# Saguaro-Biosciences/image-processing-suite

Measured on AMD Instinct MI355X. Metric: fields-of-view/sec, 2080x2080x5ch illum+seg+feat pipe, higher is better.
Workload: dtype fp32 planes / fp64 QC+features / fp32 CPnet (split-fp16 MFMA, f16x3); 1 GPU; configs[1]: 384-well plate, 1 FOV/well, 2080x2080x5ch, illum->seg->feat; batch_per_gpu=48, H=2080, W=2080, C=5, cellpose_model=nuclei, cpnet_weights=cpnet_nuclei_synth.pt, tiles_per_fov=9, parallelism=fov-sharded x1, scheduler=static per-rank steps, steps_this_rank=30, batches_in_flight_per_gpu=2

## Files before the change

### image-processing-suite_amd/csrc/cpx_internal.h

```cpp
#pragma once
#include <hip/hip_runtime.h>
#include <stdint.h>
#include <stddef.h>
#include <string>
#include <algorithm>
#include "../../include/cpx.h"

constexpr int kWsSlots = 16;

struct cpx_fov_state;

struct cpx_ctx {
  int device = 0;
  hipStream_t own_stream = nullptr;
  hipStream_t stream = nullptr;
  void* ws[kWsSlots] = {nullptr};
  size_t ws_bytes[kWsSlots] = {0};
  unsigned int ws_gen[kWsSlots] = {0};
  int n_cu = 256;
  int qc_H = 0, qc_W = 0;
  unsigned int qc_gen = 0;
  int seg_key[6] = {0, 0, 0, 0, 0, 0};
  unsigned int seg_gen = 0;
  cpx_fov_state* fov = nullptr;
// ... 64 lines not shown
template <typename T>
__device__ __forceinline__ T wave_sum(T v) {
#pragma unroll
  for (int off = 32; off > 0; off >>= 1) v += __shfl_xor(v, off, 64);
  return v;
}
template <typename T>
__device__ __forceinline__ T wave_min(T v) {
#pragma unroll
  for (int off = 32; off > 0; off >>= 1) {
    T o = __shfl_xor(v, off, 64);
    v = o < v ? o : v;
  }
  return v;
}
template <typename T>
__device__ __forceinline__ T wave_max(T v) {
#pragma unroll
  for (int off = 32; off > 0; off >>= 1) {
    T o = __shfl_xor(v, off, 64);
    v = o > v ? o : v;
  }
  return v;
}

constexpr int kClaimBroken = 1 << 30;

constexpr int kFeRegMaxLong = 128, kFeRegMaxShort = 120;
constexpr int kFeRegRows = 40;
constexpr int kFeReg1Rows = 80;
constexpr int kFeKS = 12;
constexpr int kFeU = 1;
constexpr int kFeLargeThreads = 1024, kFeLargeCells = 20224;
__host__ __device__ constexpr int fe_stride(int bw) { return (bw + 3) & ~1; }
__host__ __device__ constexpr bool fe_fits(int bh, int bw, int threads, int units, int cells) {
  const int nsr = (bh + kFeKS - 1) / kFeKS;
  return (long long)(bh + 2) * fe_stride(bw) <= cells &&
         (long long)((bw + 1) / 2) * nsr <= (long long)threads * units;
}
__host__ __device__ constexpr int fe_reg_class(int bh, int bw, bool& tr) {
  const int mn = bh < bw ? bh : bw, mx = bh < bw ? bw : bh;
  if (mn < 1) return 0;
  if (mx <= 64) { tr = bh > bw; return 1; }
  if (mn <= 64 && mx <= kFeReg1Rows) { tr = bw > bh; return 1; }
  if (mx <= 128 && mn <= 2 * kFeRegRows) { tr = bh > bw; return 2; }
  if (mx <= 128 && mn <= 3 * kFeRegRows) { tr = bh > bw; return 3; }
  return 0;
}
enum { kFeListReg1 = 0, kFeListReg2, kFeListReg3, kFeListLds, kFeListOver, kFeListUnd, kFeListFallback, kFeLists };
struct cpx_fe_lists {
  int* count;
  int2* items;
  long long cap;
  __device__ __forceinline__ int n(int l) const { return count[l]; }
  __device__ __forceinline__ int2 at(int l, int i) const { return items[l * cap + i]; }
  __device__ __forceinline__ void push(int l, int fov, int kobj) const {
    items[l * cap + atomicAdd(&count[l], 1)] = make_int2(fov, kobj);
  }
};
__host__ __device__ constexpr int fe_class(int bh, int bw) {
  bool tr = false;
  const int c = fe_reg_class(bh, bw, tr);
  if (c) return kFeListReg1 + c - 1;
  return fe_fits(bh, bw, kFeLargeThreads / 2, 2 * kFeU, kFeLargeCells) ? kFeListLds : kFeListOver;
}
static_assert(fe_class(kFeRegMaxLong, kFeRegMaxShort) == kFeListReg3 &&
                  fe_fits(kFeRegMaxLong, kFeRegMaxShort, kFeLargeThreads / 2, 2 * kFeU, kFeLargeCells) &&
                  fe_fits(kFeRegMaxShort, kFeRegMaxLong, kFeLargeThreads / 2, 2 * kFeU, kFeLargeCells),
              "register-class masks must fit the LDS screening class");

constexpr int kFastShapeWords = 4096;
__host__ __device__ inline bool cpx_shape_fits(int bh, int bw) {
  return (bh + 4) * ((bw + 4 + 31) >> 5) <= kFastShapeWords;
}
struct cpx_fallback_lists {
  int* shape;
  int* tex;
  int* n_shape;
  int* n_tex;
};
typedef int (*cpx_fallback_fn)(cpx_ctx* ctx, hipStream_t stream, const cpx_fallback_lists& fb,
                               void* arg);
int cpx_flow_error_reg_launch(int n_cu, hipStream_t stream, const int* m0, const float2* dpf, int Dy, int Dx,
                              int ML, const cpx_object* obj, cpx_fe_lists lists, int* ctr, double thr,
                              unsigned char* bad);
int cpx_features_fast(cpx_ctx* ctx, const int32_t* labels_dev, const float* corr_dev, int B, int C,
                      int H, int W, int max_label, int F, const cpx_object* objects_dev,
                      const cpx_fov_objects* hdr_dev, double* feats_dev, cpx_fallback_lists* fb,
                      cpx_fallback_fn fallback, void* fallback_arg);
int cpx_features_pair_fast(cpx_ctx* ctx, const int32_t* labels_dev, const int32_t* tlabels_dev,
                           const float* corr_dev, int B, int C, int H, int W, int max_label, int F,
                           const cpx_object* objects_dev, const cpx_fov_objects* hdr_dev, double* feats_dev,
                           const cpx_object* tobjects_dev, const cpx_fov_objects* thdr_dev, double* tfeats_dev,
                           cpx_fallback_lists* fb, cpx_fallback_lists* tfb);
```

### image-processing-suite_amd/csrc/k_flowerr_reg.hip

```cpp
#include "cpx_internal.h"
#include <math.h>
#include <stdlib.h>


#pragma clang fp contract(off)

namespace {

__device__ __forceinline__ float dpp_from_left(float v) {
  return __int_as_float(__builtin_amdgcn_mov_dpp(__float_as_int(v), 0x138, 0xf, 0xf, true));
}
__device__ __forceinline__ float dpp_from_right(float v) {
  return __int_as_float(__builtin_amdgcn_mov_dpp(__float_as_int(v), 0x130, 0xf, 0xf, true));
}

__device__ __forceinline__ int fe_hist_rank(const int* h, int len, long long k) {
  const int lane = threadIdx.x & 63;
  int e[3], s = 0;
#pragma unroll
  for (int u = 0; u < 3; ++u) {
    e[u] = 3 * lane + u < len ? h[3 * lane + u] : 0;
    s += e[u];
  }
#pragma unroll
  for (int d = 1; d < 64; d <<= 1) {
    const int y = __shfl_up(s, d, 64);
    if (lane >= d) s += y;
  }
  const unsigned long long bb = __ballot((long long)s > k);
  const int lb = bb ? __ffsll((long long)bb) - 1 : 63;
  const long long c0 = (long long)__shfl(s - e[1] - e[2], lb, 64);
  const long long c1 = c0 + __shfl(e[1], lb, 64);
  return c0 > k ? 3 * lb : c1 > k ? 3 * lb + 1 : 3 * lb + 2;
}

static_assert(3 * kFeRegRows == kFeRegMaxShort && 2 * 64 == kFeRegMaxLong, "cpx_internal.h class bounds");
typedef float fe_v2 __attribute__((ext_vector_type(2)));

template <int OP, int RW, int LO = 0, typename V>
__device__ __forceinline__ void fe_row_op(V* T, int jc, V& v) {
  if constexpr (RW - LO == 1) {
    if (jc == LO) {
      if constexpr (OP == 0) T[LO] += v;
      if constexpr (OP == 1) T[LO] = v;
      if constexpr (OP == 2) v = T[LO];
      asm volatile("; fe_row_op %0 %1" ::"n"(OP), "n"(LO));
    }
  } else {
    constexpr int MID = LO + (RW - LO) / 2;
    if (jc < MID) fe_row_op<OP, MID, LO, V>(T, jc, v);
    else fe_row_op<OP, RW, MID, V>(T, jc, v);
  }
}

constexpr int kFeReg3Rows = 32;
static_assert(4 * kFeReg3Rows >= kFeRegMaxShort, "class 3 rows fit four waves");

template <int RW, int NW, int CLS>
__global__ __launch_bounds__(64 * NW, 2) void k_flow_error_reg(
    const int* __restrict__ m0, const float2* __restrict__ dpf, int Dy, int Dx, int max_label,
    const cpx_object* __restrict__ objects, cpx_fe_lists lists, int* __restrict__ ctr, double thr,
    unsigned char* __restrict__ bad) {
  static_assert(RW % 8 == 0, "rows in groups of 8");
  constexpr int NT = 64 * NW;
  __shared__ fe_v2 xr[2][NW][2][64];
  __shared__ int hrow[RW * NW], hcol[128];
  __shared__ double sred[NW][3];
  __shared__ unsigned long long sbest[NW];
  __shared__ int sitem, smed2[2];
  const int tid = threadIdx.x, lane = tid & 63, wv = tid >> 6;
  const long long n = (long long)Dy * Dx;
  constexpr int kList = kFeListReg1 + CLS - 1;
  const int total = lists.n(kList);
  for (int claims = 0;; ++claims) {
    if (claims > total) {
      if (tid == 0) atomicOr(ctr, kClaimBroken);
      break;
    }
    if (tid == 0) sitem = atomicAdd(ctr, 1);
    __syncthreads();
    const int item = __builtin_amdgcn_readfirstlane(sitem);
    __syncthreads();
    if (item >= total) break;
    const int2 code = lists.at(kList, item);
    const int fov = code.x, kobj = code.y;
    const cpx_object o = objects[(long long)fov * max_label + kobj];
    const int L = o.label;
    const int r0 = o.bbox[0], c0 = o.bbox[1];
    const int bh = o.bbox[2] - r0, bw = o.bbox[3] - c0;
    bool tr = false;
    fe_reg_class(bh, bw, tr);
    const int SR = tr ? bw : bh, SC = tr ? bh : bw;
    const int RS = (SR + NW - 1) / NW;
    const int nrow = __builtin_amdgcn_readfirstlane(max(0, min(RS, SR - wv * RS)));
    const int* lab = m0 + (long long)fov * n + (long long)r0 * Dx + c0;
    for (int i = tid; i < RW * NW; i += NT) hrow[i] = 0;
    for (int i = tid; i < 128; i += NT) hcol[i] = 0;
    __syncthreads();
    fe_v2 T[RW], Wt[RW];
    const int gca = 2 * lane + 1, gcb = 2 * lane + 2;
    const bool ca_in = gca <= SC, cb_in = gcb <= SC;
    const int offa = tr ? (gca - 1) * Dx : gca - 1, offb = tr ? (gcb - 1) * Dx : gcb - 1;
    const int rstep = tr ? 1 : Dx;
// ... 317 lines not shown
      }
#pragma unroll
      for (int k = 0; k + 8 < RW; ++k) {
        T[k] = T[k + 8];
        Wt[k] = Wt[k + 8];
      }
#pragma unroll
      for (int k = RW - 8; k < RW; ++k) {
        T[k] = 0.f;
        Wt[k] = 0.f;
      }
    }
    e0 = wave_sum(e0);
    e1 = wave_sum(e1);
    eb = wave_sum(eb);
    if (lane == 0) {
      const double err = 0.0 + e0 / (double)o.area + e1 / (double)o.area;
      const double bnd = eb / (double)o.area + 1e-9 * (1.0 + err);
      const unsigned char v = err - thr > bnd ? 1 : thr - err > bnd ? 2 : 3;
      if (v == 3) lists.push(kFeListUnd, fov, kobj);
      bad[(long long)fov * (max_label + 1) + L] = v;
    }
  }
}


}

int cpx_flow_error_reg_launch(int n_cu, hipStream_t stream, const int* m0, const float2* dpf, int Dy, int Dx,
                              int ML, const cpx_object* obj, cpx_fe_lists lists, int* ctr, double thr,
                              unsigned char* bad) {
  hipLaunchKernelGGL((k_flow_error_reg1<kFeReg1Rows>), dim3(8 * n_cu), dim3(64), 0, stream, m0, dpf, Dy, Dx,
                     ML, obj, lists, ctr, thr, bad);
  hipLaunchKernelGGL((k_flow_error_reg<kFeRegRows, 2, 2>), dim3(4 * n_cu), dim3(128), 0, stream, m0, dpf, Dy, Dx,
                     ML, obj, lists, ctr + 1, thr, bad);
  hipLaunchKernelGGL((k_flow_error_reg<kFeReg3Rows, 4, 3>), dim3(2 * n_cu), dim3(256), 0, stream, m0, dpf, Dy, Dx,
                     ML, obj, lists, ctr + 2, thr, bad);
  CPX_CHECK_LAUNCH("k_flow_error_reg");
  return CPX_OK;
}
```

### image-processing-suite_amd/csrc/k_seg.hip

```cpp
#include "cpx_internal.h"
#include <stdlib.h>
#include <limits.h>
#include <math.h>
#include <stdio.h>
#include <type_traits>
#include <vector>

#pragma clang fp contract(off)

namespace {

constexpr int kT = 256;
constexpr int kRpad = 20;

__device__ __forceinline__ unsigned int f2key(float f) {
  unsigned int u = __float_as_uint(f);
  return (u & 0x80000000u) ? ~u : (u | 0x80000000u);
}
__device__ __forceinline__ float key2f(unsigned int k) {
  unsigned int u = (k & 0x80000000u) ? (k & 0x7fffffffu) : ~k;
  return __uint_as_float(u);
}
__device__ __forceinline__ unsigned short f2bf16(float f) {
  unsigned int u = __float_as_uint(f);
  if ((u & 0x7fffffffu) > 0x7f800000u) return 0x7fc0;
  u += 0x7fffu + ((u >> 16) & 1u);
  return (unsigned short)(u >> 16);
}
__device__ __forceinline__ float bf162f(unsigned short h) {
  return __uint_as_float(((unsigned int)h) << 16);
}

struct PctState {
// ... 823 lines not shown
  for (int j = blockIdx.x * kT + threadIdx.x; j < n_masks; j += gridDim.x * kT) {
    const int pix = d.marklist[(long long)fov * d.ms + j];
    d.mark[(long long)fov * n + pix] = 0;
    d.newlab[(long long)fov * (d.ms + 1) + d.m0[(long long)fov * n + pix]] = j + 1;
  }
  if (blockIdx.x == 0 && threadIdx.x == 0) d.st[fov].n_masks = n_masks;
}

__global__ __launch_bounds__(kT) void k_apply_newlab(int Dy, int Dx, DynBufs d) {
  const int fov = blockIdx.y;
  const long long n = (long long)Dy * Dx;
  const long long q0 = ((long long)blockIdx.x * kT + threadIdx.x) * kPx4;
  if (q0 >= n) return;
  int* m = d.m0 + (long long)fov * n;
  const int* nl = d.newlab + (long long)fov * (d.ms + 1);
  if ((n & 3) == 0 && (((uintptr_t)d.m0) & 15u) == 0) {
    const int4 t = *reinterpret_cast<const int4*>(m + q0);
    int4 o;
    o.x = t.x ? nl[t.x] : 0;
    o.y = t.y ? nl[t.y] : 0;
    o.z = t.z ? nl[t.z] : 0;
    o.w = t.w ? nl[t.w] : 0;
    *reinterpret_cast<int4*>(m + q0) = o;
  } else {
#pragma unroll
    for (int u = 0; u < kPx4; ++u)
      if (q0 + u < n) {
        const int l = m[q0 + u];
        m[q0 + u] = l ? nl[l] : 0;
      }
  }
}

template <typename E, typename E2>
__device__ __forceinline__ void fe_pair(const E2& ua, const E2& ub, const E2& ca, const E2& cb, const E2& da,
                                        const E2& db, E& n0, E& n1) {
  E s0 = ca.y + ua.y, s1 = cb.x + ub.x;
  s0 = s0 + da.y;
  s1 = s1 + db.x;
  s0 = s0 + ca.x;
  s1 = s1 + ca.y;
  s0 = s0 + cb.x;
  s1 = s1 + cb.y;
  s0 = s0 + ua.x;
  s1 = s1 + ua.y;
  s0 = s0 + ub.x;
  s1 = s1 + ub.y;
  s0 = s0 + da.x;
  s1 = s1 + da.y;
  s0 = s0 + db.x;
  s1 = s1 + db.y;
  n0 = (E)(1 / 9.) * s0;
  n1 = (E)(1 / 9.) * s1;
}

static_assert(kFeKS <= 32, "unit mask bits");

__global__ __launch_bounds__(256) void k_fe_classify(int max_label, const cpx_object* __restrict__ objects,
                                                     const cpx_fov_objects* __restrict__ hdr,
                                                     cpx_fe_lists lists) {
  const int fov = blockIdx.y, k = blockIdx.x * 256 + threadIdx.x, lane = threadIdx.x & 63;
  int cls = -1;
  if (k < min(hdr[fov].n_objects, max_label)) {
    const cpx_object& o = objects[(long long)fov * max_label + k];
    cls = fe_class(o.bbox[2] - o.bbox[0], o.bbox[3] - o.bbox[1]);
  }
  for (int c = kFeListReg1; c <= kFeListOver; ++c) {
    const unsigned long long b = __ballot(cls == c);
    if (!b) continue;
    const int lead = __ffsll((long long)b) - 1;
    int base = 0;
    if (lane == lead) base = atomicAdd(&lists.count[c], __popcll(b));
    base = __shfl(base, lead, 64);
    if (cls == c) lists.items[c * lists.cap + base + __popcll(b & ((1ull << lane) - 1ull))] = make_int2(fov, k);
  }
}

template <int THREADS>
struct FeShared {
  double sred[THREADS / 64][3];
  unsigned long long sbest[THREADS / 64];
  double smed[2];
  int sitem, stot;
};

template <int THREADS, int U, typename E>
__device__ __forceinline__ void fe_lds_mask(E* T, FeShared<THREADS>& sh, const int* __restrict__ m0,
                                            const float2* __restrict__ dpf, int Dy, int Dx, int max_label,
                                            const cpx_object* __restrict__ objects, const cpx_fe_lists& lists,
                                            int fov, int kobj, double thr, unsigned char* __restrict__ bad) {
  constexpr bool kScreen = std::is_same<E, float>::value;
  typedef typename std::conditional<kScreen, float2, double2>::type E2;
  auto& sred = sh.sred;
  auto& sbest = sh.sbest;
  auto& smed = sh.smed;
  const long long n = (long long)Dy * Dx;
  const int tid = threadIdx.x, lane = tid & 63, wid = tid >> 6;
  {
    const cpx_object o = objects[(long long)fov * max_label + kobj];
    const int L = o.label;
    const int r0 = o.bbox[0], c0 = o.bbox[1];
    const int bh = o.bbox[2] - r0, bw = o.bbox[3] - c0;
    const int ncp0 = (bw + 1) / 2;
    const int R = THREADS < 1024 ? kFeKS
                                 : min(kFeKS, max(1, (bh + max(1, THREADS * U / ncp0) - 1) / max(1, THREADS * U / ncp0)));
    const int nsr = (bh + R - 1) / R;
    const int ly = bh + 2;
    const int* lab = m0 + (long long)fov * n;
    int* rowc = reinterpret_cast<int*>(T);
    int* colc = rowc + bh;
    for (int i = tid; i < bh + bw; i += THREADS) rowc[i] = 0;
    __syncthreads();
    const int nb = bh * bw;
    for (int p = tid; p < nb; p += THREADS) {
      const int rr = p / bw, cc = p - rr * bw;
      if (lab[(long long)(r0 + rr) * Dx + c0 + cc] == L) {
        atomicAdd(&rowc[rr], 1);
        atomicAdd(&colc[cc], 1);
      }
    }
    __syncthreads();
    if (tid < 2) {
      const int* hc = tid == 0 ? rowc : colc;
      const int len = tid == 0 ? bh : bw;
      const long long cntn = o.area;
      const long long ka = (cntn - 1) / 2, kb = cntn / 2;
      long long cum = 0;
      int va = -1, vb = -1;
      for (int i = 0; i < len; ++i) {
        cum += hc[i];
        if (va < 0 && cum > ka) va = i;
        if (vb < 0 && cum > kb) { vb = i; break; }
      }
      smed[tid] = ((double)(va + 1) + (double)(vb + 1)) / 2.0;
    }
    __syncthreads();
    const double ymed = smed[0], xmed = smed[1];
    unsigned long long best = ~0ull;
    for (int p = tid; p < nb; p += THREADS) {
      const int rr = p / bw, cc = p - rr * bw;
      if (lab[(long long)(r0 + rr) * Dx + c0 + cc] != L) continue;
      const double dy = (double)(rr + 1) - ymed, dx = (double)(cc + 1) - xmed;
      const double dist = dx * dx + dy * dy;
      const unsigned long long key = ((unsigned long long)(dist * 4.0) << 32) | (unsigned int)p;
      best = key < best ? key : best;
    }
    best = wave_min(best);
    if (lane == 0) sbest[wid] = best;
    __syncthreads();
    unsigned long long bsel = sbest[0];
    for (int w = 1; w < THREADS / 64; ++w) bsel = sbest[w] < bsel ? sbest[w] : bsel;
    const int pbest = (int)(bsel & 0xffffffffu);
    const int ym = pbest / bw + 1, xm = pbest % bw + 1;
    const int niter = 2 * ((bw - 1) + (bh - 1));
    const int lxp = fe_stride(bw);
    const int ncp = (bw + 1) / 2;
    int ux[U], uy0[U], ujc[U];
    unsigned int um[U][2];
#pragma unroll
    for (int i = 0; i < U; ++i) {
      const int u = tid + i * THREADS;
      um[i][0] = um[i][1] = 0u;
      ux[i] = 1;
      uy0[i] = 1;
      ujc[i] = -1;
      if (u < ncp * nsr) {
        const int X = 2 * (u % ncp) + 1, Y0 = 1 + (u / ncp) * R;
        ux[i] = X;
        uy0[i] = Y0;
#pragma unroll
        for (int h = 0; h < 2; ++h) {
          if (X + h > bw) continue;
          unsigned int m = 0u;
          for (int j = 0; j < R && Y0 + j <= bh; ++j)
            if (lab[(long long)(r0 + Y0 - 1 + j) * Dx + c0 + X + h - 1] == L) m |= 1u << j;
          um[i][h] = m;
          if (X + h == xm && ym >= Y0 && ym < Y0 + R) ujc[i] = 2 * (ym - Y0) + h;
        }
      }
    }
    int ud[U];
#pragma unroll
    for (int i = 0; i < U; ++i)
      ud[i] = max(max(max(0, uy0[i] - ym), ym - (uy0[i] + R - 1)), max(max(0, ux[i] - xm), xm - (ux[i] + 1)));
    __syncthreads();
    for (int i = tid; i < ly * lxp; i += THREADS) T[i] = (E)0;
    __syncthreads();
    if (tid == 0 && niter > 0) T[ym * lxp + xm] = (E)1;
    __syncthreads();
    E nv[U][2][kFeKS];
    const int cidx = ym * lxp + xm;
    bool cown = false;
#pragma unroll
    for (int i = 0; i < U; ++i)
      if (ujc[i] >= 0) cown = true;
    const E2* T2 = reinterpret_cast<const E2*>(T);
    for (int it = 0; it < niter; ++it) {
#pragma unroll
      for (int i = 0; i < U; ++i) {
        if (!(um[i][0] | um[i][1]) || ud[i] > it + 1) continue;
        int r = ((uy0[i] - 1) * lxp + ux[i] - 1) >> 1;
        int rmax = ((ly - 1) * lxp + ux[i] - 1) >> 1;
        const int rs = lxp >> 1;
        asm volatile("" : "+v"(r), "+v"(rmax));
        E2 ua = T2[r], ub = T2[r + 1];
        r += rs;
        E2 ca = T2[r], cb = T2[r + 1];
        r = min(r + rs, rmax);
        E2 da = T2[r], db = T2[r + 1];
#pragma unroll
        for (int j = 0; j < kFeKS; ++j) {
          if (j < R) {
            E2 na = {(E)0, (E)0}, nb = {(E)0, (E)0};
            if (j + 1 < R) {
              r = min(r + rs, rmax);
              na = T2[r];
              nb = T2[r + 1];
            }
            fe_pair<E, E2>(ua, ub, ca, cb, da, db, nv[i][0][j], nv[i][1][j]);
            ua = ca; ub = cb;
            ca = da; cb = db;
            da = na; db = nb;
          }
          __builtin_amdgcn_sched_barrier(0);
        }
      }
      __syncthreads();
#pragma unroll
      for (int i = 0; i < U; ++i) {
        if (!(um[i][0] | um[i][1]) || ud[i] > it + 1) continue;
        int wb = uy0[i] * lxp + ux[i];
        asm volatile("" : "+v"(wb));
#pragma unroll
        for (int j = 0; j < kFeKS; ++j) {
          if ((um[i][0] >> j) & 1u) T[wb + j * lxp] = nv[i][0][j];
          if ((um[i][1] >> j) & 1u) T[wb + j * lxp + 1] = nv[i][1][j];
        }
      }
      if (cown && it + 1 < niter) T[cidx] = T[cidx] + (E)1;
      __syncthreads();
    }
    const float2* F = dpf + (long long)fov * n;
    double rho = 0.0, alpha = 0.0;
    if constexpr (kScreen) {
      const double g32 = 11.0 * 0x1p-24 * (1.0 + 1e-6), g64 = 11.0 * 0x1p-53 * (1.0 + 1e-6);
      rho = (expm1((double)niter * g32) + expm1((double)niter * g64)) / (1.0 - (double)niter * g32);
      alpha = 4.0 * (double)niter * 0x1p-126;
    }
    double e0 = 0.0, e1 = 0.0, eb = 0.0;
#pragma unroll
    for (int i = 0; i < U; ++i) {
#pragma unroll
      for (int h = 0; h < 2; ++h) {
        for (int j = 0; j < kFeKS; ++j) {
          if (!((um[i][h] >> j) & 1u)) continue;
          const int Y = uy0[i] + j, X = ux[i] + h;
          const double tdn = (double)T[(Y + 1) * lxp + X], tup = (double)T[(Y - 1) * lxp + X];
          const double trt = (double)T[Y * lxp + X + 1], tlf = (double)T[Y * lxp + X - 1];
          const double dy = tdn - tup;
          const double dx = trt - tlf;
          const double g = sqrt(dy * dy + dx * dx);
          const double nrm = 1e-20 + g;
          const double my = dy / nrm, mx = dx / nrm;
          const float2 f = F[(long long)(r0 + Y - 1) * Dx + c0 + X - 1];
          const double fy = (double)(f.x / 5.0f), fx = (double)(f.y / 5.0f);
          const double ty = my - fy;
          const double tx = mx - fx;
          e0 += ty * ty;
          e1 += tx * tx;
          if constexpr (kScreen) {
            const double Dy_ = rho * (tdn + tup) + 2.0 * alpha, Dx_ = rho * (trt + tlf) + 2.0 * alpha;
            const double D = sqrt(Dy_ * Dy_ + Dx_ * Dx_) * (1.0 + 1e-9);
            const double ff = sqrt(fy * fy + fx * fx);
            if (g > 3.0 * D && g > 1e-12) {
              const double ep = 2.0 * D / g + 1e-7;
              eb += ep * (2.0 * sqrt(ty * ty + tx * tx) + ep);
            } else {
              eb += (1.0 + ff) * (1.0 + ff);
            }
          }
        }
      }
    }
    e0 = wave_sum(e0);
    e1 = wave_sum(e1);
    if constexpr (kScreen) eb = wave_sum(eb);
    if (lane == 0) {
      sred[wid][0] = e0;
      sred[wid][1] = e1;
      sred[wid][2] = eb;
    }
    __syncthreads();
    if (tid == 0) {
      double s0 = 0.0, s1 = 0.0, sb = 0.0;
      for (int w = 0; w < THREADS / 64; ++w) {
        s0 += sred[w][0];
        s1 += sred[w][1];
        sb += sred[w][2];
      }
      const double err = 0.0 + s0 / (double)o.area + s1 / (double)o.area;
      unsigned char v = err > thr ? 1 : 2;
      if constexpr (kScreen) {
        const double bnd = sb / (double)o.area + 1e-9 * (1.0 + err);
        v = err - thr > bnd ? 1 : thr - err > bnd ? 2 : 3;
        if (v == 3) lists.push(kFeListUnd, fov, kobj);
      }
      bad[(long long)fov * (max_label + 1) + L] = v;
    }
    __syncthreads();
  }
}

template <int THREADS, int CELLS, int U, typename E, int WPE>
__global__ __launch_bounds__(THREADS, WPE) void k_flow_error_lds(
    const int* __restrict__ m0, const float2* __restrict__ dpf, int Dy, int Dx, int max_label,
    const cpx_object* __restrict__ objects, cpx_fe_lists lists, int* __restrict__ ctr, double thr,
    unsigned char* __restrict__ bad) {
  static_assert(CELLS >= kFeLargeCells && THREADS * U >= kFeLargeThreads / 2 * 2 * kFeU, "holds every mask of kFeListLds");
  __shared__ __attribute__((aligned(16))) E T[CELLS];
  __shared__ FeShared<THREADS> sh;
  const int total = lists.n(kFeListLds);
  const int tid = threadIdx.x;
  for (int claims = 0;; ++claims) {
    if (claims > total) {
      if (tid == 0) atomicOr(ctr, kClaimBroken);
      break;
    }
    if (tid == 0) sh.sitem = atomicAdd(ctr, 1);
    __syncthreads();
    const int item = sh.sitem;
    __syncthreads();
    if (item >= total) break;
    const int2 code = lists.at(kFeListLds, item);
    fe_lds_mask<THREADS, U, E>(T, sh, m0, dpf, Dy, Dx, max_label, objects, lists, code.x, code.y, thr, bad);
  }
}

constexpr int kCmpRows = 256;

template <int THREADS, int CELLS, int U>
__device__ __forceinline__ bool fe_cmp_mask(double* T, int2* rowt, FeShared<THREADS>& sh,
                                            const int* __restrict__ m0, const float2* __restrict__ dpf, int Dy,
                                            int Dx, int max_label, const cpx_object* __restrict__ objects, int fov,
                                            int kobj, double thr, unsigned char* __restrict__ bad) {
  auto& sred = sh.sred;
  auto& sbest = sh.sbest;
  auto& smed = sh.smed;
  int& stot = sh.stot;
  const long long n = (long long)Dy * Dx;
  const int tid = threadIdx.x, lane = tid & 63, wid = tid >> 6;
  const double2 z2 = {0.0, 0.0};
  {
    const cpx_object o = objects[(long long)fov * max_label + kobj];
    const int L = o.label;
    const int r0 = o.bbox[0], c0 = o.bbox[1];
    const int bh = o.bbox[2] - r0, bw = o.bbox[3] - c0;
    const int ncp = (bw + 1) / 2;
    if (bh > kCmpRows || (long long)ncp * ((bh + kFeKS - 1) / kFeKS) > (long long)THREADS * U) return false;
    const int G = max(1, THREADS * U / ncp);
    const int R = min(kFeKS, (bh + G - 1) / G);
    const int nsr = (bh + R - 1) / R;
    const int* lab = m0 + (long long)fov * n;
    int* rowc = reinterpret_cast<int*>(T);
    int* colc = rowc + bh;
    int* rmn = colc + bw;
    int* rmx = rmn + bh;
    for (int i = tid; i < bh + bw; i += THREADS) rowc[i] = 0;
// ... 1177 lines not shown
  const size_t sz_gscr = al(sizeof(double) * B * gscr_per);
  unsigned char* o = (unsigned char*)cpx_ws(ctx, WS_SEG_OBJ,
      sz_lst + sz_obj + sz_hdr + sz_bad + sz_l2i + sz_abs + sz_nl + sz_fec + sz_fel + sz_gscr);
  if (!o) return CPX_ERR_OOM;
  cpx_label_stats* lst = (cpx_label_stats*)o; o += sz_lst;
  cpx_object* obj = (cpx_object*)o; o += sz_obj;
  cpx_fov_objects* hdr = (cpx_fov_objects*)o; o += sz_hdr;
  unsigned char* bad = o; o += sz_bad;
  int* l2i = (int*)o; o += sz_l2i;
  int* absorber = (int*)o; o += sz_abs;
  int* newlab = (int*)o; o += sz_nl;
  int* fec = (int*)o; o += sz_fec;
  int2* fel = (int2*)o; o += sz_fel;
  double* gscr = (double*)o;
  ctx->fe_count_off = -1;
  if (flow_threshold > 0.0) {
    rc = cpx_objects(ctx, d.m0, B, Dy, Dx, ML, 0, lst, obj, hdr);
    if (rc) return rc;
    CPX_CHECK_HIP(hipMemsetAsync(bad, 0, sz_bad, ctx->stream));
    CPX_CHECK_HIP(hipMemsetAsync(fec, 0, sizeof(int) * (8 + kFeQueues), ctx->stream));
    const cpx_fe_lists lists = {fec, fel, (long long)B * ML};
    int* const fq = fec + 8;
    ctx->fe_count_off = (unsigned char*)fec - (unsigned char*)ctx->ws[WS_SEG_OBJ];
    hipLaunchKernelGGL(k_fe_classify, dim3(cpx_div_up(ML, 256), B), dim3(256), 0, ctx->stream, ML,
                       (const cpx_object*)obj, (const cpx_fov_objects*)hdr, lists);
    if (sev >= 0) CPX_CHECK_HIP(hipEventRecord(ctx->seg_ev[sev][2], ctx->stream));
    rc = cpx_flow_error_reg_launch(ctx->n_cu, ctx->stream, d.m0, (const float2*)d.dpf, Dy, Dx, ML, obj, lists,
                                   fq, flow_threshold, bad);
    if (rc) return rc;
    if (sev >= 0) {
      CPX_CHECK_HIP(hipEventRecord(ctx->seg_ev[sev][3], ctx->stream));
      fe_timed = true;
    }
    hipLaunchKernelGGL((k_flow_error_lds<kFeLargeThreads / 2, kFeLargeCells, 2 * kFeU, float, 4>),
                       dim3(2 * ctx->n_cu), dim3(kFeLargeThreads / 2), 0, ctx->stream, (const int*)d.m0,
                       (const float2*)d.dpf, Dy, Dx, ML, (const cpx_object*)obj, lists, fq + 3, flow_threshold,
                       bad);
    hipLaunchKernelGGL(k_flow_error_tail, dim3(ctx->n_cu), dim3(kFeLargeThreads), 0, ctx->stream,
                       (const int*)d.m0, (const float2*)d.dpf, Dy, Dx, ML, (const cpx_object*)obj, lists,
                       fq + 4, flow_threshold, bad);
    {
      const int nbig = std::max(1, std::min(ctx->n_cu, 4 * B));
      const long long slice = (long long)(B * gscr_per / nbig) & ~1LL;
      hipLaunchKernelGGL(k_flow_error_big, dim3(nbig), dim3(kBigThreads), 0, ctx->stream,
                         (const int*)d.m0, (const float2*)d.dpf, Dy, Dx, ML, (const cpx_object*)obj, lists,
                         fq + 5, flow_threshold, gscr, slice, bad);
    }
    hipLaunchKernelGGL(k_flow_error_fov, dim3(B), dim3(kFlowThreads), 0, ctx->stream,
                       (const int*)d.m0, (const float2*)d.dpf, Dy, Dx, ML, (const cpx_object*)obj, lists,
                       flow_threshold, gscr, (long long)gscr_per, bad);
    hipLaunchKernelGGL(k_apply_bad, gp4, dim3(kT), 0, ctx->stream, n, ML,
                       (const unsigned char*)bad, d.m0);
    hipLaunchKernelGGL(k_count_bad, dim3(B), dim3(256), 0, ctx->stream, ML,
                       (const unsigned char*)bad, (const int*)fq, kFeQueues, stats_dev);
    CPX_CHECK_LAUNCH("cpx_seg_masks flow error");
  }
  if (!resample) {
    hipLaunchKernelGGL(k_upsample, dim3(cpx_div_up(W, kT), cpx_div_up(H, kUpRows), B), dim3(kT), 0,
                       ctx->stream, (const int*)d.m0, Ly, Lx, H, W, tabs.ynear, tabs.xnear, labels_dev);
    CPX_CHECK_LAUNCH("k_upsample");
  }
  rc = cpx_objects(ctx, labels_dev, B, H, W, ML, 0, lst, obj, hdr);
  if (rc) return rc;
  const long long N = (long long)H * W;
  const size_t sz_fill = al(sizeof(int) * (size_t)B * N);
  const size_t sz_fscr = al(sizeof(unsigned int) * 2 * (size_t)B * ((W + 31) / 32) * H);
  unsigned char* fw = (unsigned char*)cpx_ws(ctx, WS_SEG_FILL, sz_fill + sz_fscr);
  if (!fw) return CPX_ERR_OOM;
  int* fillidx = (int*)fw;
  unsigned int* fscr = (unsigned int*)(fw + sz_fill);
// ... 38 lines not shown
```

Baseline: 501.1 FOV/s.

## Fold LDS-class flow-error screening into the class-3 register kernel

Removes the separate k_flow_error_lds launch and has the class-3 register kernel (256 threads) first drain the kFeListLds queue using a shared fp32 LDS grid, then proceed with its own register-class items. The LDS block shape changes from 512 threads x2 units to 256 threads x4 units, and the shared memory is unioned between the two phases. This saves a kernel launch and lets large masks overlap with register-class work in one persistent grid, at the cost of more LDS per block and more per-thread units, which may reduce occupancy for the class-3 path.

```diff
diff --git a/image-processing-suite_amd/csrc/cpx_internal.h b/image-processing-suite_amd/csrc/cpx_internal.h
--- a/image-processing-suite_amd/csrc/cpx_internal.h
+++ b/image-processing-suite_amd/csrc/cpx_internal.h
@@ -120,6 +120,7 @@
 constexpr int kFeKS = 12;
 constexpr int kFeU = 1;
 constexpr int kFeLargeThreads = 1024, kFeLargeCells = 20224;
+constexpr int kFeLdsThreads = 256, kFeLdsUnits = 4 * kFeU;
 __host__ __device__ constexpr int fe_stride(int bw) { return (bw + 3) & ~1; }
 __host__ __device__ constexpr bool fe_fits(int bh, int bw, int threads, int units, int cells) {
   const int nsr = (bh + kFeKS - 1) / kFeKS;
@@ -150,12 +151,13 @@
   bool tr = false;
   const int c = fe_reg_class(bh, bw, tr);
   if (c) return kFeListReg1 + c - 1;
-  return fe_fits(bh, bw, kFeLargeThreads / 2, 2 * kFeU, kFeLargeCells) ? kFeListLds : kFeListOver;
+  return fe_fits(bh, bw, kFeLdsThreads, kFeLdsUnits, kFeLargeCells) ? kFeListLds : kFeListOver;
 }
 static_assert(fe_class(kFeRegMaxLong, kFeRegMaxShort) == kFeListReg3 &&
-                  fe_fits(kFeRegMaxLong, kFeRegMaxShort, kFeLargeThreads / 2, 2 * kFeU, kFeLargeCells) &&
-                  fe_fits(kFeRegMaxShort, kFeRegMaxLong, kFeLargeThreads / 2, 2 * kFeU, kFeLargeCells),
+                  fe_fits(kFeRegMaxLong, kFeRegMaxShort, kFeLdsThreads, kFeLdsUnits, kFeLargeCells) &&
+                  fe_fits(kFeRegMaxShort, kFeRegMaxLong, kFeLdsThreads, kFeLdsUnits, kFeLargeCells),
               "register-class masks must fit the LDS screening class");
+static_assert(kFeLdsThreads * kFeLdsUnits <= kFeLargeThreads * kFeU, "kFeListLds masks fit the fp64 tail's units");
 
 constexpr int kFastShapeWords = 4096;
 __host__ __device__ inline bool cpx_shape_fits(int bh, int bw) {
diff --git a/image-processing-suite_amd/csrc/fe_lds.h b/image-processing-suite_amd/csrc/fe_lds.h
--- /dev/null
+++ b/image-processing-suite_amd/csrc/fe_lds.h
@@ -0,0 +1,267 @@
+#pragma once
+#include <type_traits>
+
+#pragma clang fp contract(off)
+
+namespace {
+
+template <typename E, typename E2>
+__device__ __forceinline__ void fe_pair(const E2& ua, const E2& ub, const E2& ca, const E2& cb, const E2& da,
+                                        const E2& db, E& n0, E& n1) {
+  E s0 = ca.y + ua.y, s1 = cb.x + ub.x;
+  s0 = s0 + da.y;
+  s1 = s1 + db.x;
+  s0 = s0 + ca.x;
+  s1 = s1 + ca.y;
+  s0 = s0 + cb.x;
+  s1 = s1 + cb.y;
+  s0 = s0 + ua.x;
+  s1 = s1 + ua.y;
+  s0 = s0 + ub.x;
+  s1 = s1 + ub.y;
+  s0 = s0 + da.x;
+  s1 = s1 + da.y;
+  s0 = s0 + db.x;
+  s1 = s1 + db.y;
+  n0 = (E)(1 / 9.) * s0;
+  n1 = (E)(1 / 9.) * s1;
+}
+
+static_assert(kFeKS <= 32, "unit mask bits");
+
+template <int THREADS>
+struct FeShared {
+  double sred[THREADS / 64][3];
+  unsigned long long sbest[THREADS / 64];
+  double smed[2];
+  int sitem, stot;
+};
+
+template <int THREADS, int U, typename E>
+__device__ __forceinline__ void fe_lds_mask(E* T, FeShared<THREADS>& sh, const int* __restrict__ m0,
+                                            const float2* __restrict__ dpf, int Dy, int Dx, int max_label,
+                                            const cpx_object* __restrict__ objects, const cpx_fe_lists& lists,
+                                            int fov, int kobj, double thr, unsigned char* __restrict__ bad) {
+  constexpr bool kScreen = std::is_same<E, float>::value;
+  typedef typename std::conditional<kScreen, float2, double2>::type E2;
+  auto& sred = sh.sred;
+  auto& sbest = sh.sbest;
+  auto& smed = sh.smed;
+  const long long n = (long long)Dy * Dx;
+  const int tid = threadIdx.x, lane = tid & 63, wid = tid >> 6;
+  {
+    const cpx_object o = objects[(long long)fov * max_label + kobj];
+    const int L = o.label;
+    const int r0 = o.bbox[0], c0 = o.bbox[1];
+    const int bh = o.bbox[2] - r0, bw = o.bbox[3] - c0;
+    const int ncp0 = (bw + 1) / 2;
+    const int R = THREADS < 1024 ? kFeKS
+                                 : min(kFeKS, max(1, (bh + max(1, THREADS * U / ncp0) - 1) / max(1, THREADS * U / ncp0)));
+    const int nsr = (bh + R - 1) / R;
+    const int ly = bh + 2;
+    const int* lab = m0 + (long long)fov * n;
+    int* rowc = reinterpret_cast<int*>(T);
+    int* colc = rowc + bh;
+    for (int i = tid; i < bh + bw; i += THREADS) rowc[i] = 0;
+    __syncthreads();
+    const int nb = bh * bw;
+    for (int p = tid; p < nb; p += THREADS) {
+      const int rr = p / bw, cc = p - rr * bw;
+      if (lab[(long long)(r0 + rr) * Dx + c0 + cc] == L) {
+        atomicAdd(&rowc[rr], 1);
+        atomicAdd(&colc[cc], 1);
+      }
+    }
+    __syncthreads();
+    if (tid < 2) {
+      const int* hc = tid == 0 ? rowc : colc;
+      const int len = tid == 0 ? bh : bw;
+      const long long cntn = o.area;
+      const long long ka = (cntn - 1) / 2, kb = cntn / 2;
+      long long cum = 0;
+      int va = -1, vb = -1;
+      for (int i = 0; i < len; ++i) {
+        cum += hc[i];
+        if (va < 0 && cum > ka) va = i;
+        if (vb < 0 && cum > kb) { vb = i; break; }
+      }
+      smed[tid] = ((double)(va + 1) + (double)(vb + 1)) / 2.0;
+    }
+    __syncthreads();
+    const double ymed = smed[0], xmed = smed[1];
+    unsigned long long best = ~0ull;
+    for (int p = tid; p < nb; p += THREADS) {
+      const int rr = p / bw, cc = p - rr * bw;
+      if (lab[(long long)(r0 + rr) * Dx + c0 + cc] != L) continue;
+      const double dy = (double)(rr + 1) - ymed, dx = (double)(cc + 1) - xmed;
+      const double dist = dx * dx + dy * dy;
+      const unsigned long long key = ((unsigned long long)(dist * 4.0) << 32) | (unsigned int)p;
+      best = key < best ? key : best;
+    }
+    best = wave_min(best);
+    if (lane == 0) sbest[wid] = best;
+    __syncthreads();
+    unsigned long long bsel = sbest[0];
+    for (int w = 1; w < THREADS / 64; ++w) bsel = sbest[w] < bsel ? sbest[w] : bsel;
+    const int pbest = (int)(bsel & 0xffffffffu);
+    const int ym = pbest / bw + 1, xm = pbest % bw + 1;
+    const int niter = 2 * ((bw - 1) + (bh - 1));
+    const int lxp = fe_stride(bw);
+    const int ncp = (bw + 1) / 2;
+    int ux[U], uy0[U], ujc[U];
+    unsigned int um[U][2];
+#pragma unroll
+    for (int i = 0; i < U; ++i) {
+      const int u = tid + i * THREADS;
+      um[i][0] = um[i][1] = 0u;
+      ux[i] = 1;
+      uy0[i] = 1;
+      ujc[i] = -1;
+      if (u < ncp * nsr) {
+        const int X = 2 * (u % ncp) + 1, Y0 = 1 + (u / ncp) * R;
+        ux[i] = X;
+        uy0[i] = Y0;
+#pragma unroll
+        for (int h = 0; h < 2; ++h) {
+          if (X + h > bw) continue;
+          unsigned int m = 0u;
+          for (int j = 0; j < R && Y0 + j <= bh; ++j)
+            if (lab[(long long)(r0 + Y0 - 1 + j) * Dx + c0 + X + h - 1] == L) m |= 1u << j;
+          um[i][h] = m;
+          if (X + h == xm && ym >= Y0 && ym < Y0 + R) ujc[i] = 2 * (ym - Y0) + h;
+        }
+      }
+    }
+    int ud[U];
+#pragma unroll
+    for (int i = 0; i < U; ++i)
+      ud[i] = max(max(max(0, uy0[i] - ym), ym - (uy0[i] + R - 1)), max(max(0, ux[i] - xm), xm - (ux[i] + 1)));
+    __syncthreads();
+    for (int i = tid; i < ly * lxp; i += THREADS) T[i] = (E)0;
+    __syncthreads();
+    if (tid == 0 && niter > 0) T[ym * lxp + xm] = (E)1;
+    __syncthreads();
+    E nv[U][2][kFeKS];
+    const int cidx = ym * lxp + xm;
+    bool cown = false;
+#pragma unroll
+    for (int i = 0; i < U; ++i)
+      if (ujc[i] >= 0) cown = true;
+    const E2* T2 = reinterpret_cast<const E2*>(T);
+    for (int it = 0; it < niter; ++it) {
+#pragma unroll
+      for (int i = 0; i < U; ++i) {
+        if (!(um[i][0] | um[i][1]) || ud[i] > it + 1) continue;
+        int r = ((uy0[i] - 1) * lxp + ux[i] - 1) >> 1;
+        int rmax = ((ly - 1) * lxp + ux[i] - 1) >> 1;
+        const int rs = lxp >> 1;
+        asm volatile("" : "+v"(r), "+v"(rmax));
+        E2 ua = T2[r], ub = T2[r + 1];
+        r += rs;
+        E2 ca = T2[r], cb = T2[r + 1];
+        r = min(r + rs, rmax);
+        E2 da = T2[r], db = T2[r + 1];
+#pragma unroll
+        for (int j = 0; j < kFeKS; ++j) {
+          if (j < R) {
+            E2 na = {(E)0, (E)0}, nb = {(E)0, (E)0};
+            if (j + 1 < R) {
+              r = min(r + rs, rmax);
+              na = T2[r];
+              nb = T2[r + 1];
+            }
+            fe_pair<E, E2>(ua, ub, ca, cb, da, db, nv[i][0][j], nv[i][1][j]);
+            ua = ca; ub = cb;
+            ca = da; cb = db;
+            da = na; db = nb;
+          }
+          __builtin_amdgcn_sched_barrier(0);
+        }
+      }
+      __syncthreads();
+#pragma unroll
+      for (int i = 0; i < U; ++i) {
+        if (!(um[i][0] | um[i][1]) || ud[i] > it + 1) continue;
+        int wb = uy0[i] * lxp + ux[i];
+        asm volatile("" : "+v"(wb));
+#pragma unroll
+        for (int j = 0; j < kFeKS; ++j) {
+          if ((um[i][0] >> j) & 1u) T[wb + j * lxp] = nv[i][0][j];
+          if ((um[i][1] >> j) & 1u) T[wb + j * lxp + 1] = nv[i][1][j];
+        }
+      }
+      if (cown && it + 1 < niter) T[cidx] = T[cidx] + (E)1;
+      __syncthreads();
+    }
+    const float2* F = dpf + (long long)fov * n;
+    double rho = 0.0, alpha = 0.0;
+    if constexpr (kScreen) {
+      const double g32 = 11.0 * 0x1p-24 * (1.0 + 1e-6), g64 = 11.0 * 0x1p-53 * (1.0 + 1e-6);
+      rho = (expm1((double)niter * g32) + expm1((double)niter * g64)) / (1.0 - (double)niter * g32);
+      alpha = 4.0 * (double)niter * 0x1p-126;
+    }
+    double e0 = 0.0, e1 = 0.0, eb = 0.0;
+#pragma unroll
+    for (int i = 0; i < U; ++i) {
+#pragma unroll
+      for (int h = 0; h < 2; ++h) {
+        for (int j = 0; j < kFeKS; ++j) {
+          if (!((um[i][h] >> j) & 1u)) continue;
+          const int Y = uy0[i] + j, X = ux[i] + h;
+          const double tdn = (double)T[(Y + 1) * lxp + X], tup = (double)T[(Y - 1) * lxp + X];
+          const double trt = (double)T[Y * lxp + X + 1], tlf = (double)T[Y * lxp + X - 1];
+          const double dy = tdn - tup;
+          const double dx = trt - tlf;
+          const double g = sqrt(dy * dy + dx * dx);
+          const double nrm = 1e-20 + g;
+          const double my = dy / nrm, mx = dx / nrm;
+          const float2 f = F[(long long)(r0 + Y - 1) * Dx + c0 + X - 1];
+          const double fy = (double)(f.x / 5.0f), fx = (double)(f.y / 5.0f);
+          const double ty = my - fy;
+          const double tx = mx - fx;
+          e0 += ty * ty;
+          e1 += tx * tx;
+          if constexpr (kScreen) {
+            const double Dy_ = rho * (tdn + tup) + 2.0 * alpha, Dx_ = rho * (trt + tlf) + 2.0 * alpha;
+            const double D = sqrt(Dy_ * Dy_ + Dx_ * Dx_) * (1.0 + 1e-9);
+            const double ff = sqrt(fy * fy + fx * fx);
+            if (g > 3.0 * D && g > 1e-12) {
+              const double ep = 2.0 * D / g + 1e-7;
+              eb += ep * (2.0 * sqrt(ty * ty + tx * tx) + ep);
+            } else {
+              eb += (1.0 + ff) * (1.0 + ff);
+            }
+          }
+        }
+      }
+    }
+    e0 = wave_sum(e0);
+    e1 = wave_sum(e1);
+    if constexpr (kScreen) eb = wave_sum(eb);
+    if (lane == 0) {
+      sred[wid][0] = e0;
+      sred[wid][1] = e1;
+      sred[wid][2] = eb;
+    }
+    __syncthreads();
+    if (tid == 0) {
+      double s0 = 0.0, s1 = 0.0, sb = 0.0;
+      for (int w = 0; w < THREADS / 64; ++w) {
+        s0 += sred[w][0];
+        s1 += sred[w][1];
+        sb += sred[w][2];
+      }
+      const double err = 0.0 + s0 / (double)o.area + s1 / (double)o.area;
+      unsigned char v = err > thr ? 1 : 2;
+      if constexpr (kScreen) {
+        const double bnd = sb / (double)o.area + 1e-9 * (1.0 + err);
+        v = err - thr > bnd ? 1 : thr - err > bnd ? 2 : 3;
+        if (v == 3) lists.push(kFeListUnd, fov, kobj);
+      }
+      bad[(long long)fov * (max_label + 1) + L] = v;
+    }
+    __syncthreads();
+  }
+}
+
+}
diff --git a/image-processing-suite_amd/csrc/k_flowerr_reg.hip b/image-processing-suite_amd/csrc/k_flowerr_reg.hip
--- a/image-processing-suite_amd/csrc/k_flowerr_reg.hip
+++ b/image-processing-suite_amd/csrc/k_flowerr_reg.hip
@@ -1,4 +1,5 @@
 #include "cpx_internal.h"
+#include "fe_lds.h"
 #include <math.h>
 #include <stdlib.h>
 
@@ -56,19 +57,59 @@
 constexpr int kFeReg3Rows = 32;
 static_assert(4 * kFeReg3Rows >= kFeRegMaxShort, "class 3 rows fit four waves");
 
-template <int RW, int NW, int CLS>
+template <int RW, int NW>
+struct FeRegShared {
+  fe_v2 xr[2][NW][2][64];
+  int hrow[RW * NW], hcol[128];
+  double sred[NW][3];
+  unsigned long long sbest[NW];
+  int sitem, smed2[2];
+};
+
+constexpr size_t kFeLdsGridBytes = sizeof(float) * kFeLargeCells;
+
+template <int RW, int NW, int CLS, bool LDSR>
 __global__ __launch_bounds__(64 * NW, 2) void k_flow_error_reg(
     const int* __restrict__ m0, const float2* __restrict__ dpf, int Dy, int Dx, int max_label,
     const cpx_object* __restrict__ objects, cpx_fe_lists lists, int* __restrict__ ctr, double thr,
     unsigned char* __restrict__ bad) {
   static_assert(RW % 8 == 0, "rows in groups of 8");
   constexpr int NT = 64 * NW;
-  __shared__ fe_v2 xr[2][NW][2][64];
-  __shared__ int hrow[RW * NW], hcol[128];
-  __shared__ double sred[NW][3];
-  __shared__ unsigned long long sbest[NW];
-  __shared__ int sitem, smed2[2];
+  typedef FeRegShared<RW, NW> RegSh;
+  constexpr size_t kLdsBytes = kFeLdsGridBytes + sizeof(FeShared<NT>);
+  constexpr size_t kShBytes = LDSR && kLdsBytes > sizeof(RegSh) ? kLdsBytes : sizeof(RegSh);
+  static_assert(!LDSR || (kShBytes <= 81920 && kFeLdsGridBytes % 16 == 0), "two blocks per CU");
+  static_assert(!LDSR || NT == kFeLdsThreads, "the block shape fe_class admits kFeListLds masks for");
+  __shared__ __attribute__((aligned(16))) unsigned char smem[kShBytes];
   const int tid = threadIdx.x, lane = tid & 63, wv = tid >> 6;
+  if constexpr (LDSR) {
+    float* Tl = reinterpret_cast<float*>(smem);
+    FeShared<NT>& sh = *reinterpret_cast<FeShared<NT>*>(smem + kFeLdsGridBytes);
+    int* const lctr = ctr + 1;
+    const int ltotal = lists.n(kFeListLds);
+    for (int claims = 0;; ++claims) {
+      if (claims > ltotal) {
+        if (tid == 0) atomicOr(lctr, kClaimBroken);
+        break;
+      }
+      if (tid == 0) sh.sitem = atomicAdd(lctr, 1);
+      __syncthreads();
+      const int item = __builtin_amdgcn_readfirstlane(sh.sitem);
+      __syncthreads();
+      if (item >= ltotal) break;
+      const int2 code = lists.at(kFeListLds, item);
+      fe_lds_mask<NT, kFeLdsUnits, float>(Tl, sh, m0, dpf, Dy, Dx, max_label, objects, lists, code.x, code.y, thr,
+                                          bad);
+    }
+  }
+  RegSh& rs = *reinterpret_cast<RegSh*>(smem);
+  auto& xr = rs.xr;
+  auto& hrow = rs.hrow;
+  auto& hcol = rs.hcol;
+  auto& sred = rs.sred;
+  auto& sbest = rs.sbest;
+  auto& smed2 = rs.smed2;
+  int& sitem = rs.sitem;
   const long long n = (long long)Dy * Dx;
   constexpr int kList = kFeListReg1 + CLS - 1;
   const int total = lists.n(kList);
@@ -452,10 +493,10 @@
                               unsigned char* bad) {
   hipLaunchKernelGGL((k_flow_error_reg1<kFeReg1Rows>), dim3(8 * n_cu), dim3(64), 0, stream, m0, dpf, Dy, Dx,
                      ML, obj, lists, ctr, thr, bad);
-  hipLaunchKernelGGL((k_flow_error_reg<kFeRegRows, 2, 2>), dim3(4 * n_cu), dim3(128), 0, stream, m0, dpf, Dy, Dx,
-                     ML, obj, lists, ctr + 1, thr, bad);
-  hipLaunchKernelGGL((k_flow_error_reg<kFeReg3Rows, 4, 3>), dim3(2 * n_cu), dim3(256), 0, stream, m0, dpf, Dy, Dx,
-                     ML, obj, lists, ctr + 2, thr, bad);
+  hipLaunchKernelGGL((k_flow_error_reg<kFeRegRows, 2, 2, false>), dim3(4 * n_cu), dim3(128), 0, stream, m0, dpf,
+                     Dy, Dx, ML, obj, lists, ctr + 1, thr, bad);
+  hipLaunchKernelGGL((k_flow_error_reg<kFeReg3Rows, 4, 3, true>), dim3(2 * n_cu), dim3(256), 0, stream, m0, dpf,
+                     Dy, Dx, ML, obj, lists, ctr + 2, thr, bad);
   CPX_CHECK_LAUNCH("k_flow_error_reg");
   return CPX_OK;
 }
diff --git a/image-processing-suite_amd/csrc/k_seg.hip b/image-processing-suite_amd/csrc/k_seg.hip
--- a/image-processing-suite_amd/csrc/k_seg.hip
+++ b/image-processing-suite_amd/csrc/k_seg.hip
@@ -1,4 +1,5 @@
 #include "cpx_internal.h"
+#include "fe_lds.h"
 #include <stdlib.h>
 #include <limits.h>
 #include <math.h>
@@ -888,29 +889,6 @@
   }
 }
 
-template <typename E, typename E2>
-__device__ __forceinline__ void fe_pair(const E2& ua, const E2& ub, const E2& ca, const E2& cb, const E2& da,
-                                        const E2& db, E& n0, E& n1) {
-  E s0 = ca.y + ua.y, s1 = cb.x + ub.x;
-  s0 = s0 + da.y;
-  s1 = s1 + db.x;
-  s0 = s0 + ca.x;
-  s1 = s1 + ca.y;
-  s0 = s0 + cb.x;
-  s1 = s1 + cb.y;
-  s0 = s0 + ua.x;
-  s1 = s1 + ua.y;
-  s0 = s0 + ub.x;
-  s1 = s1 + ub.y;
-  s0 = s0 + da.x;
-  s1 = s1 + da.y;
-  s0 = s0 + db.x;
-  s1 = s1 + db.y;
-  n0 = (E)(1 / 9.) * s0;
-  n1 = (E)(1 / 9.) * s1;
-}
-
-static_assert(kFeKS <= 32, "unit mask bits");
 
 __global__ __launch_bounds__(256) void k_fe_classify(int max_label, const cpx_object* __restrict__ objects,
                                                      const cpx_fov_objects* __restrict__ hdr,
@@ -929,266 +907,6 @@
     if (lane == lead) base = atomicAdd(&lists.count[c], __popcll(b));
     base = __shfl(base, lead, 64);
     if (cls == c) lists.items[c * lists.cap + base + __popcll(b & ((1ull << lane) - 1ull))] = make_int2(fov, k);
-  }
-}
-
-template <int THREADS>
-struct FeShared {
-  double sred[THREADS / 64][3];
-  unsigned long long sbest[THREADS / 64];
-  double smed[2];
-  int sitem, stot;
-};
-
-template <int THREADS, int U, typename E>
-__device__ __forceinline__ void fe_lds_mask(E* T, FeShared<THREADS>& sh, const int* __restrict__ m0,
-                                            const float2* __restrict__ dpf, int Dy, int Dx, int max_label,
-                                            const cpx_object* __restrict__ objects, const cpx_fe_lists& lists,
-                                            int fov, int kobj, double thr, unsigned char* __restrict__ bad) {
-  constexpr bool kScreen = std::is_same<E, float>::value;
-  typedef typename std::conditional<kScreen, float2, double2>::type E2;
-  auto& sred = sh.sred;
-  auto& sbest = sh.sbest;
-  auto& smed = sh.smed;
-  const long long n = (long long)Dy * Dx;
-  const int tid = threadIdx.x, lane = tid & 63, wid = tid >> 6;
-  {
-    const cpx_object o = objects[(long long)fov * max_label + kobj];
-    const int L = o.label;
-    const int r0 = o.bbox[0], c0 = o.bbox[1];
-    const int bh = o.bbox[2] - r0, bw = o.bbox[3] - c0;
-    const int ncp0 = (bw + 1) / 2;
-    const int R = THREADS < 1024 ? kFeKS
-                                 : min(kFeKS, max(1, (bh + max(1, THREADS * U / ncp0) - 1) / max(1, THREADS * U / ncp0)));
-    const int nsr = (bh + R - 1) / R;
-    const int ly = bh + 2;
-    const int* lab = m0 + (long long)fov * n;
-    int* rowc = reinterpret_cast<int*>(T);
-    int* colc = rowc + bh;
-    for (int i = tid; i < bh + bw; i += THREADS) rowc[i] = 0;
-    __syncthreads();
-    const int nb = bh * bw;
-    for (int p = tid; p < nb; p += THREADS) {
-      const int rr = p / bw, cc = p - rr * bw;
-      if (lab[(long long)(r0 + rr) * Dx + c0 + cc] == L) {
-        atomicAdd(&rowc[rr], 1);
-        atomicAdd(&colc[cc], 1);
-      }
-    }
-    __syncthreads();
-    if (tid < 2) {
-      const int* hc = tid == 0 ? rowc : colc;
-      const int len = tid == 0 ? bh : bw;
-      const long long cntn = o.area;
-      const long long ka = (cntn - 1) / 2, kb = cntn / 2;
-      long long cum = 0;
-      int va = -1, vb = -1;
-      for (int i = 0; i < len; ++i) {
-        cum += hc[i];
-        if (va < 0 && cum > ka) va = i;
-        if (vb < 0 && cum > kb) { vb = i; break; }
-      }
-      smed[tid] = ((double)(va + 1) + (double)(vb + 1)) / 2.0;
-    }
-    __syncthreads();
-    const double ymed = smed[0], xmed = smed[1];
-    unsigned long long best = ~0ull;
-    for (int p = tid; p < nb; p += THREADS) {
-      const int rr = p / bw, cc = p - rr * bw;
-      if (lab[(long long)(r0 + rr) * Dx + c0 + cc] != L) continue;
-      const double dy = (double)(rr + 1) - ymed, dx = (double)(cc + 1) - xmed;
-      const double dist = dx * dx + dy * dy;
-      const unsigned long long key = ((unsigned long long)(dist * 4.0) << 32) | (unsigned int)p;
-      best = key < best ? key : best;
-    }
-    best = wave_min(best);
-    if (lane == 0) sbest[wid] = best;
-    __syncthreads();
-    unsigned long long bsel = sbest[0];
-    for (int w = 1; w < THREADS / 64; ++w) bsel = sbest[w] < bsel ? sbest[w] : bsel;
-    const int pbest = (int)(bsel & 0xffffffffu);
-    const int ym = pbest / bw + 1, xm = pbest % bw + 1;
-    const int niter = 2 * ((bw - 1) + (bh - 1));
-    const int lxp = fe_stride(bw);
-    const int ncp = (bw + 1) / 2;
-    int ux[U], uy0[U], ujc[U];
-    unsigned int um[U][2];
-#pragma unroll
-    for (int i = 0; i < U; ++i) {
-      const int u = tid + i * THREADS;
-      um[i][0] = um[i][1] = 0u;
-      ux[i] = 1;
-      uy0[i] = 1;
-      ujc[i] = -1;
-      if (u < ncp * nsr) {
-        const int X = 2 * (u % ncp) + 1, Y0 = 1 + (u / ncp) * R;
-        ux[i] = X;
-        uy0[i] = Y0;
-#pragma unroll
-        for (int h = 0; h < 2; ++h) {
-          if (X + h > bw) continue;
-          unsigned int m = 0u;
-          for (int j = 0; j < R && Y0 + j <= bh; ++j)
-            if (lab[(long long)(r0 + Y0 - 1 + j) * Dx + c0 + X + h - 1] == L) m |= 1u << j;
-          um[i][h] = m;
-          if (X + h == xm && ym >= Y0 && ym < Y0 + R) ujc[i] = 2 * (ym - Y0) + h;
-        }
-      }
-    }
-    int ud[U];
-#pragma unroll
-    for (int i = 0; i < U; ++i)
-      ud[i] = max(max(max(0, uy0[i] - ym), ym - (uy0[i] + R - 1)), max(max(0, ux[i] - xm), xm - (ux[i] + 1)));
-    __syncthreads();
-    for (int i = tid; i < ly * lxp; i += THREADS) T[i] = (E)0;
-    __syncthreads();
-    if (tid == 0 && niter > 0) T[ym * lxp + xm] = (E)1;
-    __syncthreads();
-    E nv[U][2][kFeKS];
-    const int cidx = ym * lxp + xm;
-    bool cown = false;
-#pragma unroll
-    for (int i = 0; i < U; ++i)
-      if (ujc[i] >= 0) cown = true;
-    const E2* T2 = reinterpret_cast<const E2*>(T);
-    for (int it = 0; it < niter; ++it) {
-#pragma unroll
-      for (int i = 0; i < U; ++i) {
-        if (!(um[i][0] | um[i][1]) || ud[i] > it + 1) continue;
-        int r = ((uy0[i] - 1) * lxp + ux[i] - 1) >> 1;
-        int rmax = ((ly - 1) * lxp + ux[i] - 1) >> 1;
-        const int rs = lxp >> 1;
-        asm volatile("" : "+v"(r), "+v"(rmax));
-        E2 ua = T2[r], ub = T2[r + 1];
-        r += rs;
-        E2 ca = T2[r], cb = T2[r + 1];
-        r = min(r + rs, rmax);
-        E2 da = T2[r], db = T2[r + 1];
-#pragma unroll
-        for (int j = 0; j < kFeKS; ++j) {
-          if (j < R) {
-            E2 na = {(E)0, (E)0}, nb = {(E)0, (E)0};
-            if (j + 1 < R) {
-              r = min(r + rs, rmax);
-              na = T2[r];
-              nb = T2[r + 1];
-            }
-            fe_pair<E, E2>(ua, ub, ca, cb, da, db, nv[i][0][j], nv[i][1][j]);
-            ua = ca; ub = cb;
-            ca = da; cb = db;
-            da = na; db = nb;
-          }
-          __builtin_amdgcn_sched_barrier(0);
-        }
-      }
-      __syncthreads();
-#pragma unroll
-      for (int i = 0; i < U; ++i) {
-        if (!(um[i][0] | um[i][1]) || ud[i] > it + 1) continue;
-        int wb = uy0[i] * lxp + ux[i];
-        asm volatile("" : "+v"(wb));
-#pragma unroll
-        for (int j = 0; j < kFeKS; ++j) {
-          if ((um[i][0] >> j) & 1u) T[wb + j * lxp] = nv[i][0][j];
-          if ((um[i][1] >> j) & 1u) T[wb + j * lxp + 1] = nv[i][1][j];
-        }
-      }
-      if (cown && it + 1 < niter) T[cidx] = T[cidx] + (E)1;
-      __syncthreads();
-    }
-    const float2* F = dpf + (long long)fov * n;
-    double rho = 0.0, alpha = 0.0;
-    if constexpr (kScreen) {
-      const double g32 = 11.0 * 0x1p-24 * (1.0 + 1e-6), g64 = 11.0 * 0x1p-53 * (1.0 + 1e-6);
-      rho = (expm1((double)niter * g32) + expm1((double)niter * g64)) / (1.0 - (double)niter * g32);
-      alpha = 4.0 * (double)niter * 0x1p-126;
-    }
-    double e0 = 0.0, e1 = 0.0, eb = 0.0;
-#pragma unroll
-    for (int i = 0; i < U; ++i) {
-#pragma unroll
-      for (int h = 0; h < 2; ++h) {
-        for (int j = 0; j < kFeKS; ++j) {
-          if (!((um[i][h] >> j) & 1u)) continue;
-          const int Y = uy0[i] + j, X = ux[i] + h;
-          const double tdn = (double)T[(Y + 1) * lxp + X], tup = (double)T[(Y - 1) * lxp + X];
-          const double trt = (double)T[Y * lxp + X + 1], tlf = (double)T[Y * lxp + X - 1];
-          const double dy = tdn - tup;
-          const double dx = trt - tlf;
-          const double g = sqrt(dy * dy + dx * dx);
-          const double nrm = 1e-20 + g;
-          const double my = dy / nrm, mx = dx / nrm;
-          const float2 f = F[(long long)(r0 + Y - 1) * Dx + c0 + X - 1];
-          const double fy = (double)(f.x / 5.0f), fx = (double)(f.y / 5.0f);
-          const double ty = my - fy;
-          const double tx = mx - fx;
-          e0 += ty * ty;
-          e1 += tx * tx;
-          if constexpr (kScreen) {
-            const double Dy_ = rho * (tdn + tup) + 2.0 * alpha, Dx_ = rho * (trt + tlf) + 2.0 * alpha;
-            const double D = sqrt(Dy_ * Dy_ + Dx_ * Dx_) * (1.0 + 1e-9);
-            const double ff = sqrt(fy * fy + fx * fx);
-            if (g > 3.0 * D && g > 1e-12) {
-              const double ep = 2.0 * D / g + 1e-7;
-              eb += ep * (2.0 * sqrt(ty * ty + tx * tx) + ep);
-            } else {
-              eb += (1.0 + ff) * (1.0 + ff);
-            }
-          }
-        }
-      }
-    }
-    e0 = wave_sum(e0);
-    e1 = wave_sum(e1);
-    if constexpr (kScreen) eb = wave_sum(eb);
-    if (lane == 0) {
-      sred[wid][0] = e0;
-      sred[wid][1] = e1;
-      sred[wid][2] = eb;
-    }
-    __syncthreads();
-    if (tid == 0) {
-      double s0 = 0.0, s1 = 0.0, sb = 0.0;
-      for (int w = 0; w < THREADS / 64; ++w) {
-        s0 += sred[w][0];
-        s1 += sred[w][1];
-        sb += sred[w][2];
-      }
-      const double err = 0.0 + s0 / (double)o.area + s1 / (double)o.area;
-      unsigned char v = err > thr ? 1 : 2;
-      if constexpr (kScreen) {
-        const double bnd = sb / (double)o.area + 1e-9 * (1.0 + err);
-        v = err - thr > bnd ? 1 : thr - err > bnd ? 2 : 3;
-        if (v == 3) lists.push(kFeListUnd, fov, kobj);
-      }
-      bad[(long long)fov * (max_label + 1) + L] = v;
-    }
-    __syncthreads();
-  }
-}
-
-template <int THREADS, int CELLS, int U, typename E, int WPE>
-__global__ __launch_bounds__(THREADS, WPE) void k_flow_error_lds(
-    const int* __restrict__ m0, const float2* __restrict__ dpf, int Dy, int Dx, int max_label,
-    const cpx_object* __restrict__ objects, cpx_fe_lists lists, int* __restrict__ ctr, double thr,
-    unsigned char* __restrict__ bad) {
-  static_assert(CELLS >= kFeLargeCells && THREADS * U >= kFeLargeThreads / 2 * 2 * kFeU, "holds every mask of kFeListLds");
-  __shared__ __attribute__((aligned(16))) E T[CELLS];
-  __shared__ FeShared<THREADS> sh;
-  const int total = lists.n(kFeListLds);
-  const int tid = threadIdx.x;
-  for (int claims = 0;; ++claims) {
-    if (claims > total) {
-      if (tid == 0) atomicOr(ctr, kClaimBroken);
-      break;
-    }
-    if (tid == 0) sh.sitem = atomicAdd(ctr, 1);
-    __syncthreads();
-    const int item = sh.sitem;
-    __syncthreads();
-    if (item >= total) break;
-    const int2 code = lists.at(kFeListLds, item);
-    fe_lds_mask<THREADS, U, E>(T, sh, m0, dpf, Dy, Dx, max_label, objects, lists, code.x, code.y, thr, bad);
   }
 }
 
@@ -2432,10 +2150,6 @@
       CPX_CHECK_HIP(hipEventRecord(ctx->seg_ev[sev][3], ctx->stream));
       fe_timed = true;
     }
-    hipLaunchKernelGGL((k_flow_error_lds<kFeLargeThreads / 2, kFeLargeCells, 2 * kFeU, float, 4>),
-                       dim3(2 * ctx->n_cu), dim3(kFeLargeThreads / 2), 0, ctx->stream, (const int*)d.m0,
-                       (const float2*)d.dpf, Dy, Dx, ML, (const cpx_object*)obj, lists, fq + 3, flow_threshold,
-                       bad);
     hipLaunchKernelGGL(k_flow_error_tail, dim3(ctx->n_cu), dim3(kFeLargeThreads), 0, ctx->stream,
                        (const int*)d.m0, (const float2*)d.dpf, Dy, Dx, ML, (const cpx_object*)obj, lists,
                        fq + 4, flow_threshold, bad);
```

Measured after the change: 503.8 FOV/s (median of 6 runs). No clear change (+0.5%).
